# Animesh005/Torus-FHE

Measured on AMD Instinct MI355X. Metric: bootstrapped gates/sec (NAND, N=1024), higher is better.
Workload: dtype f64

## Files before the change

torus-fhe_amd/csrc/thfhe_common.h:

```cpp
#ifndef THFHE_COMMON_H
#define THFHE_COMMON_H

#include <hip/hip_runtime.h>

#include <type_traits>

#include "../../include/thfhe_hip.h"
#include "thfhe_lane.h"

namespace thfhe {

constexpr int kOpIdentity = 100;

int thfhe_fail(int code, const char *msg);
int thfhe_fail_hip(hipError_t e, const char *what);

inline int ilog2(int x) {
    int l = 0;
    while ((1 << l) < x) l++;
    return l;
}

inline int lut_validate(const thfhe_lut_spec *sp, const void *tv, int n_luts, const int32_t *lut_index, const int32_t *in0, const int32_t *in1,
                        const int32_t *in2, const int32_t *out, size_t count, int max_luts = 1024) {
// ... 125 lines not shown
                w[r + 1][d] = __builtin_amdgcn_update_dpp(b, a, 0x128, 0xF, 0x3, false);
                w[r][d] = __builtin_amdgcn_update_dpp(a, b, 0x128, 0xF, 0xC, false);
            }
        }
    }
    if constexpr (KEEP64) {
#pragma unroll
        for (int r = 0; r < 8; r += 2) {
#pragma unroll
            for (int k = 0; k < 2; k++) {
                uint64_t keep = (uint64_t)w[r + 1][2 * k] | (uint64_t)w[r + 1][2 * k + 1] << 32;
                asm("" : "+v"(keep));
#pragma unroll
                for (int h = 0; h < 2; h++) {
                    const int d = 2 * k + h;
                    const uint32_t a = w[r][d], b = w[r + 1][d], kept = (uint32_t)(keep >> (32 * h));
                    w[r + 1][d] = __builtin_amdgcn_update_dpp(b, a, 0x128, 0xF, 0x3, false);
                    w[r][d] = __builtin_amdgcn_update_dpp(a, kept, 0x128, 0xF, 0xC, false);
                }
            }
        }
    }
#pragma unroll
    for (int r = 0; r < 8; r++) __builtin_memcpy(&z[r], w[r], 16);
}
__device__ __forceinline__ void wave_fft_fwd_q(int lane, cplx (&z)[8], cplx *xb, const LaneRoots &r, const W64 &w) {
    fwdq_seg1(z, r);
    wave_transpose_hi3(z);
    wave_sync();
    fwdr_seg2_st(lane, z, xb, w);
    wave_sync();
    fwd_seg3(lane, z, xb);
}
template <bool FLIPPED>
__device__ __forceinline__ void wave_transpose_x3(cplx (&z)[8]) {
    uint32_t w[8][4];
#pragma unroll
    for (int r = 0; r < 8; r++) __builtin_memcpy(w[r], &z[r], 16);
    if constexpr (FLIPPED) {
#pragma unroll
        for (int r = 4; r < 8; r++)
#pragma unroll
            for (int d = 0; d < 4; d++) w[r][d] = __builtin_amdgcn_update_dpp(w[r][d], w[r][d], 0x128, 0xF, 0xF, false);
    } else {
#pragma unroll
        for (int r = 0; r < 4; r++) {
#pragma unroll
            for (int k = 0; k < 2; k++) {
                uint64_t keep = (uint64_t)w[r + 4][2 * k] | (uint64_t)w[r + 4][2 * k + 1] << 32;
                asm("" : "+v"(keep));
#pragma unroll
                for (int h = 0; h < 2; h++) {
                    const int d = 2 * k + h;
                    const uint32_t a = w[r][d], b = w[r + 4][d], kept = (uint32_t)(keep >> (32 * h));
                    w[r + 4][d] = __builtin_amdgcn_update_dpp(b, a, 0x128, 0xF, 0x3, false);
                    w[r][d] = __builtin_amdgcn_update_dpp(a, kept, 0x128, 0xF, 0xC, false);
                }
            }
        }
    }
#pragma unroll
    for (int d = 0; d < 4; d++) {
#pragma unroll
        for (int r = 0; r < 8; r++) {
            if (r & 2) continue;
            auto q = __builtin_amdgcn_permlane32_swap(w[r][d], w[r + 2][d], false, false);
            w[r][d] = q[0];
            w[r + 2][d] = q[1];
        }
#pragma unroll
        for (int r = 0; r < 8; r += 2) {
            auto q = __builtin_amdgcn_permlane16_swap(w[r][d], w[r + 1][d], false, false);
            w[r][d] = q[0];
            w[r + 1][d] = q[1];
        }
    }
#pragma unroll
    for (int r = 0; r < 8; r++) __builtin_memcpy(&z[r], w[r], 16);
}
__device__ __forceinline__ void wave_fft_fwd_x(int lane, cplx (&z)[8], cplx *xb, const LaneRootsF &r) {
    fwdf_seg1(z);
    wave_transpose_x3<false>(z);
    wave_sync();
    fwdx_seg2_st(lane, z, xb, r);
    wave_sync();
    fwdf_seg3(lane, z, xb, r);
}
template <bool LEAN>
__device__ __forceinline__ void wave_fft_inv_x(int lane, cplx (&z)[8], cplx *xb, W64 &w, LaneRoots &r, uint32_t flip, const cplx (&bc)[4]) {
    if (LEAN) opaque_in_place(w.w1), opaque_in_place(r.s);
    wave_sync();
    invf_seg1(lane, z, xb);
    wave_sync();
    inv_seg2_ld(lane, z, xb);
    invf_seg2(z, w);
    wave_transpose_x3<true>(z);
    invx_seg3(z, r, flip, bc);
}
__device__ __forceinline__ void wave_fft_fwd_qs(int lane, cplx (&z)[8], cplx *xb, const LaneRoots &r, const W64 &w) {
    fwdq_seg1(z, r);
    wave_transpose_hi3(z);
    wave_sync();
    fwds_seg2_st(lane, z, xb, w);
    wave_sync();
    fwds_seg3(lane, z, xb);
}
__device__ __forceinline__ void wave_fft_inv_qs(int lane, cplx (&z)[8], cplx *xb, const LaneRoots &r, const W64 &w) {
    wave_sync();
    invs_seg1(lane, z, xb, w);
    wave_sync();
    invs_seg2_ld(lane, z, xb);
    dft8<-1>(z);
    wave_transpose_hi3(z);
    invq_seg3(z, r);
}
template <int T>
__device__ __forceinline__ void wave_fft_fwd_t(int lane, cplx (&z)[8], cplx *xb, const cplx *T1t, const W64 &w) {
    wave_sync();
    fwdt_seg1<T>(lane, z, xb, T1t);
    wave_sync();
    fwds_seg2_ld(lane, z, xb);
    fwds_seg2_st(lane, z, xb, w);
    wave_sync();
    fwds_seg3(lane, z, xb);
}
template <int T>
__device__ __forceinline__ void wave_fft_inv_t(int lane, cplx (&z)[8], cplx *xb, const cplx *T1t, const W64 &w) {
    wave_sync();
    invs_seg1(lane, z, xb, w);
    wave_sync();
// ... 62 lines not shown
```

torus-fhe_amd/csrc/thfhe_lane.h:

```cpp
#ifndef THFHE_LANE_H
#define THFHE_LANE_H

#include <limits.h>
#include <stddef.h>
#include <stdint.h>

#if defined(__HIPCC__)
#define THFHE_FN __host__ __device__ __forceinline__
#else
#define THFHE_FN inline __attribute__((always_inline))
#endif

namespace thfhe {

constexpr int kLanes = 64;
constexpr int kXbufSlots = 8 * 72;

struct alignas(16) cplx {
    double re, im;
};

THFHE_FN cplx cmul(cplx a, cplx b) { return cplx{a.re * b.re - a.im * b.im, a.re * b.im + a.im * b.re}; }
THFHE_FN cplx cmul_conj(cplx a, cplx b) {
    return cplx{a.re * b.re + a.im * b.im, a.im * b.re - a.re * b.im};
// ... 349 lines not shown
}
THFHE_FN W64 lane_w64_x(cplx w64_j0, uint32_t flip) { return W64{cplx{flip_sign(w64_j0.re, flip), flip_sign(w64_j0.im, flip)}}; }
template <typename WPtr>
THFHE_FN LaneRoots lane_roots_x(const WPtr tw, int t1_base, int roots_base, int lane) {
    const int nu = lane_nu(lane);
    return LaneRoots{(lane & 8) ? tw[t1_base + 4 * 64 + nu] : tw[roots_base + 2 * nu], tw[roots_base + 2 * nu + 1]};
}
THFHE_FN void make_untwist_x(cplx b, uint32_t flip, cplx (&bc)[4]) {
    make_untwist_f(b, bc);
    bc[1] = cplx{flip_sign(bc[1].re, flip), flip_sign(bc[1].im, flip)};
    bc[3] = cplx{flip_sign(bc[3].re, flip), flip_sign(bc[3].im, flip)};
}
THFHE_FN constexpr int fwdx_phys(int j1) { return ((j1 & 1) << 2) | ((j1 >> 2) & 1) << 1 | ((j1 >> 1) & 1); }
THFHE_FN void fwdx_seg2_st(int lane, cplx (&z)[8], cplx *xbuf, const LaneRootsF &r) {
    cplx y[8];
#pragma unroll
    for (int j1 = 0; j1 < 8; j1++) y[j1] = z[fwdx_phys(j1)];
    dft8_tw<+1>(y, root_powers<+1>(r.s));
#pragma unroll
    for (int k1 = 0; k1 < 8; k1++) xbuf[xs_c(k1, lane)] = y[k1];
}
THFHE_FN void invx_seg3(cplx (&z)[8], const LaneRoots &r, uint32_t flip, const cplx (&bc)[4]) {
    constexpr double R = 0.70710678118654752440;
    RootPow p = root_powers<-1>(cconj(r.s));
    p.w4.im = flip_sign(p.w4.im, flip);
    dft8_tw<-1>(z, p);
#pragma unroll
    for (int m = 0; m < 4; m++) {
        z[m] = cmul_conj(z[m], bc[m]);
        z[m + 4] = cmul_conj(cplx{R * (z[m + 4].re + z[m + 4].im), R * (z[m + 4].im - z[m + 4].re)}, bc[m]);
    }
}

THFHE_FN uint32_t rot_minus_self32(const int32_t *p, int q, int a2n, int N) {
    int e = (q - a2n) & (2 * N - 1);
    uint32_t r = (uint32_t)p[e & (N - 1)];
    if (e & N) r = 0u - r;
    return r - (uint32_t)p[q];
}
THFHE_FN double digit32(uint32_t v, int shift, uint32_t mask, int32_t half) {
    return (double)((int32_t)((v >> shift) & mask) - half);
}
THFHE_FN uint32_t decomp_offset32(int l, int Bgbit) {
    uint32_t off = 0;
    for (int p = 1; p <= l; p++) off += (1u << (Bgbit - 1)) << (32 - p * Bgbit);
    return off;
}
THFHE_FN uint32_t round_lo32(double x) {
    double y = x + 6755399441055744.0;
    uint64_t b;
    __builtin_memcpy(&b, &y, 8);
    return (uint32_t)b;
}
THFHE_FN void split_limbs32(int32_t v, double &lo, double &hi) {
    int32_t l = (int32_t)(int16_t)(uint16_t)v;
    int32_t h = (int32_t)(((int64_t)v - l) >> 16);
    lo = (double)l;
    hi = (double)h;
}

THFHE_FN int32_t modswitch2n(int32_t x, int log2_2n) {
    int32_t y = (int32_t)((uint32_t)x + (1u << (32 - log2_2n - 1)));
    return y >> (32 - log2_2n);
}


// ... 153 lines not shown
    s.im = __builtin_fma(z.im, b.re, s.im);
}
THFHE_FN void cfma_negkey(cplx &s, cplx z, cplx b) {
    s.re = __builtin_fma(z.re, b.re, s.re);
    s.im = __builtin_fma(z.re, b.im, s.im);
    s.re = __builtin_fma(z.im, -b.im, s.re);
    s.im = __builtin_fma(z.im, b.re, s.im);
}
template <int DEPTH = 8>
THFHE_FN void mac8(int lane, cplx (&S)[8], const cplx (&z)[8], const cplx *B) {
#pragma unroll
    for (int m0 = 0; m0 < 8; m0 += DEPTH) {
        cplx b[DEPTH];
#pragma unroll
        for (int q = 0; q < DEPTH; q++) b[q] = B[(m0 + q) * 64 + lane];
#pragma unroll
        for (int q = 0; q < DEPTH; q++) cfma(S[m0 + q], z[m0 + q], b[q]);
    }
}
THFHE_FN void load8(int lane, cplx (&b)[8], const cplx *B) {
#pragma unroll
    for (int m = 0; m < 8; m++) b[m] = B[m * 64 + lane];
}
THFHE_FN void mac8r(cplx (&S)[8], const cplx (&z)[8], const cplx (&b)[8]) {
#pragma unroll
    for (int m = 0; m < 8; m++) cfma(S[m], z[m], b[m]);
}
THFHE_FN void acc_update16(int lane, int32_t *acc_poly, const cplx (&zlo)[8], const cplx (&zhi)[8]) {
#pragma unroll
    for (int m = 0; m < 8; m++) {
        int q = lane + 64 * m;
        uint32_t vr = round_lo32(zlo[m].re) + (round_lo32(zhi[m].re) << 16);
        uint32_t vi = round_lo32(zlo[m].im) + (round_lo32(zhi[m].im) << 16);
        acc_poly[q] = (int32_t)((uint32_t)acc_poly[q] + vr);
        acc_poly[q + 512] = (int32_t)((uint32_t)acc_poly[q + 512] + vi);
    }
}
THFHE_FN void acc_init16(int lane, int32_t *acc_mask, int32_t *acc_body, int barb, int32_t mu) {
#pragma unroll
    for (int m = 0; m < 16; m++) {
        int q = lane + 64 * m;
        int e = (q + barb) & 2047;
        acc_mask[q] = 0;
        acc_body[q] = (e & 1024) ? (int32_t)(0u - (uint32_t)mu) : mu;
    }
}
THFHE_FN void extract16(int lane, const int32_t *acc_mask, const int32_t *acc_body, int32_t *out) {
#pragma unroll
    for (int m = 0; m < 16; m++) {
        int q = lane + 64 * m;
        out[q] = q == 0 ? acc_mask[0] : (int32_t)(0u - (uint32_t)acc_mask[1024 - q]);
    }
    if (lane == 0) out[1024] = acc_body[0];
}
THFHE_FN void acc_init_tv16(int lane, int32_t *acc_mask, int32_t *acc_body, int barb, const int32_t *tv) {
#pragma unroll
    for (int m = 0; m < 16; m++) {
        int q = lane + 64 * m;
        int e = (q + barb) & 2047;
        const int32_t v = tv[e & 1023];
        acc_mask[q] = 0;
        acc_body[q] = (e & 1024) ? (int32_t)(0u - (uint32_t)v) : v;
    }
}
THFHE_FN void acc_init_tlwe16(int lane, int32_t *acc_mask, int32_t *acc_body, int barb, const int32_t *tv_a, const int32_t *tv_b) {
#pragma unroll
// ... 60 lines not shown
THFHE_FN uint64_t decomp_offset64(int l, int Bgbit) {
    uint64_t off = 0;
    for (int p = 1; p <= l; p++) off += (1ull << (Bgbit - 1)) << (64 - p * Bgbit);
    return off;
}
THFHE_FN void load_rotated16_hi(int lane, const int64_t *acc_poly, int a2n, uint64_t offset, uint32_t (&t)[16]) {
#pragma unroll
    for (int m = 0; m < 16; m++) t[m] = (uint32_t)((rot_minus_self64(acc_poly, lane + 64 * m, a2n) + offset) >> 32);
}
THFHE_FN void split_limbs64(int64_t v, double (&l)[4]) {
#pragma unroll
    for (int q = 0; q < 3; q++) {
        int64_t lo = (int64_t)(int16_t)(uint16_t)v;
        l[q] = (double)lo;
        v = (v - lo) >> 16;
    }
    l[3] = (double)v;
}
template <int TB>
THFHE_FN cplx limb_pair(const void *poly, int q0, int q1, int h) {
    if (TB == 32) {
        const int32_t *p = static_cast<const int32_t *>(poly);
        double l0, h0, l1, h1;
        split_limbs32(p[q0], l0, h0);
        split_limbs32(p[q1], l1, h1);
        return h == 0 ? cplx{l0, l1} : cplx{h0, h1};
    } else {
        const int64_t *p = static_cast<const int64_t *>(poly);
        double a[4], b[4];
        split_limbs64(p[q0], a);
        split_limbs64(p[q1], b);
        return cplx{a[h], b[h]};
    }
}
THFHE_FN void key_limbs64_to_z(int lane, const int64_t *poly, cplx (&z)[4][8]) {
#pragma unroll
    for (int h = 0; h < 4; h++)
#pragma unroll
        for (int m = 0; m < 8; m++) z[h][m] = limb_pair<64>(poly, lane + 64 * m, lane + 64 * m + 512, h);
}
THFHE_FN void key_limbs64_to_z16(int lane, const int64_t *poly, int h, cplx (&z)[16]) {
#pragma unroll
    for (int m = 0; m < 16; m++) z[m] = limb_pair<64>(poly, lane + 64 * m, lane + 64 * m + 1024, h);
}
THFHE_FN int64_t round_i64(double x) {
    double y = x + 6755399441055744.0;
    int64_t b;
    __builtin_memcpy(&b, &y, 8);
    return b - 0x4338000000000000ll;
}
THFHE_FN void acc_update16_64(int lane, int64_t *acc_poly, const cplx (&S)[4][8]) {
#pragma unroll
    for (int m = 0; m < 8; m++) {
        int q = lane + 64 * m;
        uint64_t vr = 0, vi = 0;
#pragma unroll
        for (int h = 0; h < 4; h++) {
            vr += (uint64_t)round_i64(S[h][m].re) << (16 * h);
            vi += (uint64_t)round_i64(S[h][m].im) << (16 * h);
        }
        acc_poly[q] = (int64_t)((uint64_t)acc_poly[q] + vr);
        acc_poly[q + 512] = (int64_t)((uint64_t)acc_poly[q + 512] + vi);
    }
}
THFHE_FN void acc_init16_64(int lane, int64_t *acc_mask, int64_t *acc_body, int barb, int64_t mu) {
#pragma unroll
// ... 319 lines not shown
```

torus-fhe_amd/csrc/thfhe_sk.hip:

```cpp
#include <hip/hip_runtime.h>

#include <algorithm>
#include <memory>
#include <mutex>
#include <new>
#include <string>
#include <vector>

#include "../../include/thfhe_hip.h"
#include "thfhe_cb.h"
#include "thfhe_common.h"
#include "thfhe_dag.h"
#include "thfhe_devctx.h"
#include "thfhe_keyswitch.h"
#include "thfhe_lane.h"
#include "thfhe_launch_plan.h"
#include "thfhe_pack.h"
#include "thfhe_pbs_host.h"
#include "thfhe_ring_schedule.h"

using namespace thfhe;

namespace {

// ... 18 lines not shown
    case THFHE_ORYN: L = Lin{E8, 1, -1, 1}; return true;
    case THFHE_MUX: L = which == 0 ? Lin{-E8, 1, 1, 1} : Lin{-E8, -1, 1, 2}; return true;
    case kOpIdentity: L = Lin{0, 1, 0, 1}; return true;
    default: return false;
    }
}

__global__ __launch_bounds__(256) void sk_prologue_kernel(const int32_t *__restrict__ in0, const int32_t *__restrict__ in1,
                                                           const int32_t *__restrict__ in2, int op, const int32_t *__restrict__ ops,
                                                           int rot_per_gate, int n, int n_pad, int log2_2n, long jobs,
                                                           int32_t *__restrict__ bara, int32_t *__restrict__ barb) {
    const long job = blockIdx.y;
    const int i = blockIdx.x * 256 + threadIdx.x;
    if (job >= jobs || i > n) return;
    const long gate = job / rot_per_gate;
    const int which = (int)(job % rot_per_gate);
    Lin L;
    gate_lin(ops ? ops[gate] : op, which, L);
    const size_t off = (size_t)gate * (n + 1) + i;
    uint32_t v = (uint32_t)L.cx * (uint32_t)in0[off];
    if (L.cy != 0) v += (uint32_t)L.cy * (uint32_t)(L.ysel == 2 ? in2[off] : in1[off]);
    if (i == n) {
        v += (uint32_t)L.cb;
        barb[job] = modswitch2n((int32_t)v, log2_2n);
    } else {
        bara[job * n_pad + i] = modswitch2n((int32_t)v, log2_2n);
    }
}

THFHE_STAMP_STORAGE

struct BRArgs {
    const cplx *bk;
    const cplx *tw;
    const int32_t *bara;
    const int32_t *barb;
    int32_t *out;
    long jobs;
    int n, n_pad, Bgbit;
    int32_t mu;
    const int32_t *tv;
    const int32_t *lut_idx;
    int theta;
    const int32_t *tv_a;
    const int32_t *mv_w;
    int mv_p, mv_box;
};

constexpr int kGate = 0, kLut = 1, kLutEnc = 2, kLutMv = 3;

template <int L, int W = 8, int LUT = kGate>
__global__ __launch_bounds__(64 * W, W == 8 ? 2 : 1) void sk_blind_rotate_ring_kernel(BRArgs a) {
    __shared__ __attribute__((aligned(4096))) int32_t sAcc[W][2048];
    __shared__ cplx sX[W][kXbufSlots];
    __shared__ cplx sRing[3][512];
    constexpr int ROWS = 2 * L;
    constexpr int DPC = 8 / W;
    namespace RS = ring_schedule;
    const int wave = __builtin_amdgcn_readfirstlane(threadIdx.x >> 6);
    const int lane = threadIdx.x & 63;
    const int nu = lane_nu(lane);
    const uint32_t flip = lane_flip_x(lane);
    W64 w64 = lane_w64_x(a.tw[TwRing1k::T2 + 1 * 8 + (lane & 7)], flip);
    LaneRoots roots = lane_roots_x(a.tw, TwRing1k::T1, TwRing1k::ROOTS, lane);
    LaneRootsF rootsf{a.tw[TwRing1k::ROOTSF + 2 * nu], a.tw[TwRing1k::ROOTSF + 2 * nu + 1]};
    const long job = (long)blockIdx.x * W + wave;
    const bool has_job = job < a.jobs;
    int32_t *acc = sAcc[wave];
    cplx *xb = sX[wave];
    const uniform_i32_ptr bara = as_uniform(a.bara + (has_job ? job : 0) * a.n_pad);
    const int Bgbit = a.Bgbit;
    if (has_job) {
        if constexpr (LUT == kLutEnc) {
            const size_t t = a.lut_idx ? (size_t)a.lut_idx[job] * 1024 : 0;
            acc_init_tlwe16(lane, acc, acc + 1024, a.barb[job], a.tv_a + t, a.tv + t);
        } else if constexpr (LUT == kLutMv) acc_init_tv16(lane, acc, acc + 1024, a.barb[job], a.tv);
        else if constexpr (LUT) acc_init_tv16(lane, acc, acc + 1024, a.barb[job], a.tv + (a.lut_idx ? (size_t)a.lut_idx[job] * 1024 : 0));
        else acc_init16(lane, acc, acc + 1024, a.barb[job], a.mu);
    }

    static_assert(DPC == 1 || DPC == 2, "a wave brings one slice of a chunk, or two 1 KiB apart");
    const uint32_t lane_off = (uint32_t)(wave * (64 * DPC) + lane) * (uint32_t)sizeof(cplx);
    uint64_t gbase = (uint64_t)(size_t)a.bk;
    int chunks_ahead = a.n * ROWS * RS::kChunksPerRow - 1;
    asm volatile("" : "+s"(gbase), "+s"(chunks_ahead));
    static_assert(RS::kResidentSlots * RS::kSlotBytes == sizeof(sRing) && RS::kSlotBytes <= sizeof(sX[0]), "ring schedule against the LDS layout");
    const uint32_t ring_base = (uint32_t)(size_t)(__attribute__((address_space(3))) void *)&sRing[0][0] + (uint32_t)wave * (1024u * DPC);
    const uint32_t lent_base = (uint32_t)(size_t)(__attribute__((address_space(3))) void *)&sX[0][0] + (uint32_t)wave * (1024u * DPC);
    auto issue = [&](int slot) {
        const uint32_t dst = slot == RS::kBorrowedSlot ? lent_base : ring_base + (uint32_t)slot * (uint32_t)RS::kSlotBytes;
        ring_dma(gbase, lane_off, dst);
        if constexpr (DPC == 2) ring_dma<1024>(gbase, lane_off, dst);
        gbase += chunks_ahead > 0 ? (uint32_t)RS::kSlotBytes : 0u;
        chunks_ahead = chunks_ahead > 0 ? chunks_ahead - 1 : 0;
    };
    auto slot_ptr = [&](int slot) -> const cplx * { return slot == RS::kBorrowedSlot ? &sX[0][0] : &sRing[slot][0]; };
    __syncthreads();
#pragma unroll
    for (int k = 0; k < RS::kPrologueIssues; k++) issue(RS::kPlan[k].slot);
    STAMP_DECL;

    for (int i = 0; i < a.n; i++) {
        const int ai = bara[i];
        const bool active = has_job && ai != 0;
        const int a2n = ai & 2047;
        cplx S[2][2][8];
#pragma unroll
        for (int c = 0; c < 2; c++)
#pragma unroll
            for (int h = 0; h < 2; h++)
#pragma unroll
                for (int m = 0; m < 8; m++) S[c][h][m] = cplx{0.0, 0.0};
        constexpr int NF = 16;
        uint32_t fld[NF];
#pragma unroll
        for (int r = 0; r < ROWS; r++) {
            cplx z[8];
            if (active) {
                int a2n_r = a2n;
                asm volatile("" : "+s"(a2n_r));
                if (r % L == 0) rotated_fields_keep<NF, W == 4>(lane, acc + (r / L) * 1024, a2n_r, L, Bgbit, fld);
                asm volatile("" : "+s"(a2n_r));
                mixed_digits_z<NF>(lane, acc + (r / L) * 1024, a2n_r, (r % L) + 1, L, Bgbit, fld, z);
                if (W == 8) opaque_in_place(rootsf.s), opaque_in_place(rootsf.w);
                wave_fft_fwd_x(lane, z, xb, rootsf);
            }
            STAMP(0);
            cplx bA[4], bB[4];
            auto consume = [&](int c4) {
                const cplx *B = slot_ptr(RS::kPlan[c4].slot);
                if (active) {
#pragma unroll
                    for (int m = 0; m < 4; m++) bA[m] = B[m * 64 + nu];
                    if (c4 > 0) {
#pragma unroll
                        for (int m = 0; m < 4; m++) cfma_negkey(S[(c4 - 1) >> 1][(c4 - 1) & 1][4 + m], z[4 + m], bB[m]);
                    }
#pragma unroll
                    for (int m = 0; m < 4; m++) bB[m] = B[(4 + m) * 64 + nu];
#pragma unroll
                    for (int m = 0; m < 4; m++) cfma_negkey(S[c4 >> 1][c4 & 1][m], z[m], bA[m]);
                }
            };
            ring_barrier<RS::vmcnt_at(RS::kBarA) * DPC>();
            STAMP(1);
#pragma unroll
            for (int k = 0; k < RS::issues_at(RS::kBarA); k++) issue(RS::issue_slot(RS::kBarA, k));
#pragma unroll
            for (int c4 = RS::first_consumed(RS::kBarA); c4 < RS::first_consumed(RS::kBarX); c4++) consume(c4);
            STAMP(2);
            ring_barrier<RS::vmcnt_at(RS::kBarX) * DPC>();
            STAMP(1);
#pragma unroll
            for (int k = 0; k < RS::issues_at(RS::kBarX); k++) issue(RS::issue_slot(RS::kBarX, k));
#pragma unroll
            for (int c4 = RS::first_consumed(RS::kBarX); c4 < RS::first_consumed(RS::kBarB); c4++) consume(c4);
            STAMP(2);
            ring_barrier<RS::vmcnt_at(RS::kBarB) * DPC>();
            static_assert(RS::issues_at(RS::kBarB) == 0 && RS::first_consumed(RS::kBarB) == RS::kChunksPerRow, "nothing is issued or read after barrier B");
            STAMP(1);
            if (active) {
#pragma unroll
                for (int m = 0; m < 4; m++) cfma_negkey(S[1][1][4 + m], z[4 + m], bB[m]);
            }
            STAMP(2);
        }
        if (active) {
            wave_sync();
            cplx bc[4];
            if (W == 8) opaque_in_place(roots.b);
            make_untwist_x(roots.b, flip, bc);
#pragma unroll
            for (int c = 0; c < 2; c++) {
                wave_fft_inv_x<W == 8>(lane, S[c][0], xb, w64, roots, flip, bc);
                wave_fft_inv_x<W == 8>(lane, S[c][1], xb, w64, roots, flip, bc);
                acc_update16(nu, acc + c * 1024, S[c][0], S[c][1]);
            }
            wave_sync();
        }
        STAMP(3);
    }
    STAMP_FLUSH(blockIdx.x, wave);
    asm volatile("s_waitcnt vmcnt(0)" ::: "memory");
    if (has_job) {
        if constexpr (LUT == kLutMv) {
            const uniform_i32_ptr w = as_uniform(a.mv_w) + (size_t)(a.lut_idx ? as_uniform(a.lut_idx)[job] : 0) * a.theta * a.mv_p;
            for (int j = 0; j < a.theta; j++) extract_mv16(lane, acc, acc + 1024, w + j * a.mv_p, a.mv_p, a.mv_box, a.out + (job * a.theta + j) * 1025);
        } else if constexpr (LUT) {
            for (int j = 0; j < a.theta; j++) extract_at16(lane, acc, acc + 1024, j, a.out + (job * a.theta + j) * 1025);
        } else {
            extract16(lane, acc, acc + 1024, a.out + job * 1025);
        }
    }
}

__device__ __forceinline__ void wg_barrier() { asm volatile("s_waitcnt lgkmcnt(0)\n\ts_barrier" ::: "memory"); }
__device__ __forceinline__ void pin() { asm volatile("" ::: "memory"); }

template <int L, int LUT = kGate>
__global__ __launch_bounds__(512, 2) void sk_blind_rotate_coop_kernel(BRArgs a) {
    constexpr int ROWS = 2 * L;
    __shared__ __attribute__((aligned(4096))) int32_t sAcc[2048];
    __shared__ cplx sSpec[ROWS][512];
    __shared__ cplx sX[8][kXbufSlots];
    const int wave = __builtin_amdgcn_readfirstlane(threadIdx.x >> 6);
    const int lane = threadIdx.x & 63;
    const W64 w64{a.tw[TwRing1k::T2 + 1 * 8 + (lane & 7)]};
    const LaneRoots roots{a.tw[TwRing1k::ROOTS + 2 * lane], a.tw[TwRing1k::ROOTS + 2 * lane + 1]};
    const long job = blockIdx.x;
// ... 103 lines not shown
        STAMP(5);
        i = inext;
    }
    STAMP_FLUSH(blockIdx.x, wave);
    if constexpr (LUT == kLutMv) {
        const uniform_i32_ptr w = as_uniform(a.mv_w) + (size_t)(a.lut_idx ? as_uniform(a.lut_idx)[job] : 0) * a.theta * a.mv_p;
        for (int j = wave; j < a.theta; j += 8)
            extract_mv16(lane, sAcc, sAcc + 1024, w + j * a.mv_p, a.mv_p, a.mv_box, a.out + (job * a.theta + j) * 1025);
    } else if constexpr (LUT) {
        if (wave < a.theta) extract_at16(lane, sAcc, sAcc + 1024, wave, a.out + (job * a.theta + wave) * 1025);
    } else {
        if (wave == 0) extract16(lane, sAcc, sAcc + 1024, a.out + job * 1025);
    }
}

__global__ __launch_bounds__(256) void sk_linear_kernel(const int32_t *__restrict__ in0, int32_t *__restrict__ out, size_t words, int negate) {
    const size_t q = (size_t)blockIdx.x * 256 + threadIdx.x;
    if (q < words) out[q] = negate ? (int32_t)(0u - (uint32_t)in0[q]) : in0[q];
}

}

struct THFHE_INTERNAL thfhe_tgsw_set {
    thfhe_ctx *ctx = nullptr;
    DevBuf spec;
    size_t count = 0;
    int d = 0;
};

struct THFHE_INTERNAL thfhe_ctx : DevCtx {
    thfhe_params p;
    int rec_words() const { return p.n + 1; }
    DevBuf d_bk;
    KsKey ksk;
    int coop_max_jobs = 768;
    int ring4_max_jobs = 1024;
    int n_pad = 0;
    DevBuf d_bara, d_barb, d_u;
    DevBuf d_tv, d_lut_idx;
    DevBuf d_tva;
    DevBuf d_mv_w;
    DevBuf d_tree_tab, d_tree_lwe, d_tree_a, d_tree_b;
    DevBuf d_dag_enc_a, d_dag_enc_b, d_dag_tv1;
    DevBuf d_dag_mv_tv0, d_dag_mv_w;
    DevBuf d_dag_lhe_tab_a, d_dag_lhe_tab_b, d_dag_lhe_fin_a, d_dag_lhe_fin_b, d_dag_lhe_words;
    DevBuf d_lhe_a, d_lhe_b, d_lhe_in[4];
    DevBuf d_wfa_tab;
    DevBuf d_sc_tab, d_sc_idx;
    CbKey cb;
    std::vector<std::unique_ptr<thfhe_tgsw_set>> cb_sets;
    std::vector<const thfhe_tgsw_set *> dag_sets;
    DevBuf d_cb_lwe, d_cb_bara, d_cb_barb, d_cb_acc, d_cb_x, d_cb_lwe2, d_cb_rows, d_cb_tv;
    int cus = 0;
    int wfa_chunk = 0;
    size_t tree_slice = 65536;
    Stage stage;
    LinBufs lin;
    DagBuffers dag;
    size_t dag_slice = 28672;
    hipEvent_t grp_ev[2] = {nullptr, nullptr};
    bool grp_valid = false;
    ~thfhe_ctx() {
        for (hipEvent_t e : grp_ev)
            if (e) (void)hipEventDestroy(e);
    }
};
// ... 25 lines not shown
    auto piece = [&](long first, long count) {
        BRArgs b = a;
        b.bara += first * a.n_pad, b.barb += first, b.jobs = count;
        b.out += first * (LUT ? a.theta : 1) * 1025;
        if (LUT && b.lut_idx) b.lut_idx += first;
        return b;
    };
    launch_plan::SkPiece pc[launch_plan::kMaxPieces];
    const int n = launch_plan::sk_rotation_plan(a.jobs, coop_max, ring4_max, pc);
    for (int i = 0; i < n; i++) {
        const BRArgs b = piece(pc[i].first, pc[i].count);
        if (pc[i].shape == launch_plan::kRing8) launch_ring8<L, LUT>(b, s);
        else if (pc[i].shape == launch_plan::kCoop) launch_coop<L, LUT>(b, s);
        else launch_ring4<L, LUT>(b, s);
    }
}

template <int LUT>
int launch_rotations(thfhe_ctx *c, const BRArgs &a) {
    return with_static_int<4>(c->p.l, kBadL, [&](auto l) { launch_br<decltype(l)::value, LUT>(a, c->stream, c->coop_max_jobs, c->ring4_max_jobs); });
}

int enqueue_rotations(thfhe_ctx *c, int op, const int32_t *d0, const int32_t *d1, const int32_t *d2, size_t gates,
                      int rot_per_gate, int32_t mu, const int32_t *d_ops = nullptr) {
    const size_t jobs = gates * rot_per_gate;
    int rc = ensure_workspace(c, jobs);
    if (rc) return rc;
    const int n = c->p.n;
    if (c->profiling) THFHE_HIP(hipEventRecord(c->ev[0], c->stream));
    dim3 pg((unsigned)((n + 1 + 255) / 256), (unsigned)jobs);
    hipLaunchKernelGGL(sk_prologue_kernel, pg, dim3(256), 0, c->stream, d0, d1, d2, op, d_ops, rot_per_gate, n, c->n_pad,
                       ilog2(2 * c->p.N), (long)jobs, c->d_bara.as<int32_t>(), c->d_barb.as<int32_t>());
    if (c->profiling) THFHE_HIP(hipEventRecord(c->ev[1], c->stream));
    BRArgs a{c->d_bk.as<cplx>(), c->d_tw.as<cplx>(), c->d_bara.as<int32_t>(), c->d_barb.as<int32_t>(), c->d_u.as<int32_t>(), (long)jobs, n, c->n_pad, c->p.Bgbit, mu};
    rc = launch_rotations<kGate>(c, a);
    if (rc) return rc;
    if (c->profiling) THFHE_HIP(hipEventRecord(c->ev[2], c->stream));
    THFHE_HIP(hipGetLastError());
    return THFHE_OK;
}

int enqueue_keyswitch(thfhe_ctx *c, const int32_t *d_u, int32_t *d_out, size_t gates, int rot_per_gate, bool timed) {
    KsArgs k = c->ksk.args(d_u, d_out, (long)gates);
    k.rot_per_gate = rot_per_gate;
    const int nsplit = gates <= 32 ? 16 : (gates <= 128 ? 8 : (gates <= 512 ? 2 : 1));
    THFHE_TRY(ks_enqueue(c->ksk, k, nsplit, c->stream));
    if (timed && c->profiling) {
        THFHE_HIP(hipEventRecord(c->ev[3], c->stream));
        c->ev_valid = true;
    }
    return THFHE_OK;
}

struct MvArgs {
    const int32_t *w;
    int p;
};

template <typename Src>
int enqueue_pbs(thfhe_ctx *c, const Src &src, size_t jobs, const int32_t *tv, const int32_t *tv_a, int theta, const int32_t *d_idx, int32_t *ks_dst,
                bool timed = false, const MvArgs *mv = nullptr) {
    const int n = c->p.n;
    const bool ev = timed && c->profiling;
    int32_t *const idx = c->d_lut_idx.as<int32_t>();
    if (ev) THFHE_HIP(hipEventRecord(c->ev[0], c->stream));
    lut_prologue_launch(src, jobs, n, c->n_pad, ilog2(2 * c->p.N), c->d_bara.as<int32_t>(), c->d_barb.as<int32_t>(), idx, c->stream);
    if (ev) THFHE_HIP(hipEventRecord(c->ev[1], c->stream));
    BRArgs a{c->d_bk.as<cplx>(), c->d_tw.as<cplx>(), c->d_bara.as<int32_t>(), c->d_barb.as<int32_t>(), c->d_u.as<int32_t>(), (long)jobs, n, c->n_pad, c->p.Bgbit,
             0, tv, Src::kIdx == LutIdx::none ? d_idx : idx, theta, tv_a};
    if (mv) {
        a.mv_w = mv->w, a.mv_p = mv->p, a.mv_box = c->p.N / mv->p;
        THFHE_TRY(launch_rotations<kLutMv>(c, a));
    } else THFHE_TRY(tv_a ? launch_rotations<kLutEnc>(c, a) : launch_rotations<kLut>(c, a));
    if (ev) THFHE_HIP(hipEventRecord(c->ev[2], c->stream));
    THFHE_HIP(hipGetLastError());
    return ks_dst ? enqueue_keyswitch(c, c->d_u.as<int32_t>(), ks_dst, jobs * theta, 1, timed) : THFHE_OK;
}

int gates_dev_locked(thfhe_ctx *c, int op, const int32_t *d0, const int32_t *d1, const int32_t *d2, int32_t *dout, size_t count) {
    if (count == 0) return THFHE_OK;
    if (count > (size_t)INT32_MAX / 4) return thfhe_fail(THFHE_E_INVALID, "count too large");
    THFHE_HIP(hipSetDevice(c->device));
    if (op == THFHE_NOT || op == THFHE_COPY) {
        const size_t words = count * c->rec_words();
        hipLaunchKernelGGL(sk_linear_kernel, dim3((unsigned)((words + 255) / 256)), dim3(256), 0, c->stream, d0, dout, words,
                           op == THFHE_NOT ? 1 : 0);
        THFHE_HIP(hipGetLastError());
        return THFHE_OK;
    }
    Lin L;
    if (!gate_lin(op, 0, L) || op == kOpIdentity) return thfhe_fail(THFHE_E_INVALID, "unknown gate opcode");
    if (!d0 || !d1 || (op == THFHE_MUX && !d2)) return thfhe_fail(THFHE_E_INVALID, "null operand");
    const int rot = op == THFHE_MUX ? 2 : 1;
    int rc = enqueue_rotations(c, op, d0, d1, d2, count, rot, 1 << 29);
    if (rc) return rc;
    return enqueue_keyswitch(c, c->d_u.as<int32_t>(), dout, count, rot, true);
}

int dag_gate_class(thfhe_ctx *c, int cls, const int32_t *d_ops, size_t n) {
    const bool is_mux = cls == kDagMux;
    int r = enqueue_rotations(c, is_mux ? THFHE_MUX : THFHE_NAND, c->stage.in_ptr(0), c->stage.in_ptr(1), is_mux ? c->stage.in_ptr(2) : nullptr, n, is_mux ? 2 : 1, 1 << 29,
// ... 253 lines not shown
int thfhe_device_count(void) {
    int n = 0;
    if (hipGetDeviceCount(&n) != hipSuccess) return 0;
    return n;
}

int thfhe_device_pci_bus_id(int device, char *buf, int len) {
    if (!buf || len < 16) return thfhe_fail(THFHE_E_INVALID, "buffer of at least 16 bytes expected");
    THFHE_HIP(hipDeviceGetPCIBusId(buf, len, device));
    return THFHE_OK;
}

int thfhe_ctx_create(const thfhe_params *p, const int32_t *bk_coeff, const int32_t *ksk, int device, thfhe_ctx **out) {
    if (!p || !bk_coeff || !ksk || !out) return thfhe_fail(THFHE_E_INVALID, "null argument");
    *out = nullptr;
    if (p->torus_bits != 32 || p->parties != 1) return thfhe_fail(THFHE_E_UNSUPPORTED, "thfhe_ctx_create is the single-key Torus32 path; use thfhe_mk_ctx_create");
    if (p->N != 1024 || p->k != 1) return thfhe_fail(THFHE_E_UNSUPPORTED, "only N = 1024, k = 1 is implemented");
    if (p->l < 1 || p->l > 4 || p->Bgbit < 1 || p->Bgbit > 10 || p->l * p->Bgbit > 32)
        return thfhe_fail(THFHE_E_UNSUPPORTED, "need 1 <= l <= 4, Bgbit <= 10 (FP64 exactness bound), l*Bgbit <= 32");
    if (p->n < 1 || p->n > 1407) return thfhe_fail(THFHE_E_UNSUPPORTED, "need 1 <= n <= 1407");
    if (p->ks_t < 1 || p->ks_basebit < 1 || p->ks_t * p->ks_basebit > 31) return thfhe_fail(THFHE_E_INVALID, "bad key-switch parameters");
    std::unique_ptr<thfhe_ctx> c(new (std::nothrow) thfhe_ctx);
    if (!c) return thfhe_fail(THFHE_E_NOMEM, "out of host memory");
    THFHE_TRY(c->open(device, true));
    c->p = *p;
    c->n_pad = (p->n + 3) & ~3;
    THFHE_TRY(c->upload_twiddles(1024));
    DevBuf coeff;
    const long npolys = (long)p->n * 2 * p->l * 2;
    THFHE_TRY(coeff.grow((size_t)npolys * 1024 * sizeof(int32_t)));
    THFHE_HIP(hipMemcpyAsync(coeff.as<int32_t>(), bk_coeff, (size_t)npolys * 1024 * sizeof(int32_t), hipMemcpyHostToDevice, c->stream));
    THFHE_TRY(c->d_bk.grow((size_t)npolys * 1024 * sizeof(cplx)));
    THFHE_TRY((launch_torus_transform<1024, 32>(c->stream, coeff.as<int32_t>(), npolys, c->d_tw.as<cplx>(), c->d_bk.as<cplx>())));
    THFHE_TRY(c->ksk.upload(ksk, 1, p->N, p->n, p->ks_t, p->ks_basebit, true, c->stream));
    *out = c.release();
    return THFHE_OK;
}

void thfhe_ctx_destroy(thfhe_ctx *c) { ctx_destroy(c); }

int thfhe_ctx_params(const thfhe_ctx *c, thfhe_params *out) {
    if (!c || !out) return thfhe_fail(THFHE_E_INVALID, "null argument");
    *out = c->p;
    return THFHE_OK;
}

void *thfhe_dev_alloc(thfhe_ctx *c, size_t bytes) { return ctx_dev_alloc(c, bytes); }
void thfhe_dev_free(thfhe_ctx *c, void *p) { ctx_dev_free(c, p); }
int thfhe_copy_h2d(thfhe_ctx *c, void *dst, const void *src, size_t bytes) { return ctx_copy(c, dst, src, bytes, hipMemcpyHostToDevice); }
int thfhe_copy_d2h(thfhe_ctx *c, void *dst, const void *src, size_t bytes) { return ctx_copy(c, dst, src, bytes, hipMemcpyDeviceToHost); }
int thfhe_reserve(thfhe_ctx *c, size_t max_count) {
    if (!c) return thfhe_fail(THFHE_E_INVALID, "null ctx");
    DevLock lk(*c);
    if (lk.rc) return lk.rc;
    return ensure_workspace(c, max_count * 2);
}
int thfhe_sync(thfhe_ctx *c) { return ctx_sync(c); }
#ifdef THFHE_STAMPS
int thfhe_debug_read_stamps(unsigned long long *dst, size_t count) {
    return hipMemcpyFromSymbol(dst, HIP_SYMBOL(g_stamps), count * sizeof(unsigned long long)) == hipSuccess ? 0 : -1;
}
#endif
int thfhe_set_coop_threshold(thfhe_ctx *c, int max_jobs) {
    if (!c || max_jobs < 0) return thfhe_fail(THFHE_E_INVALID, "bad argument");
    std::lock_guard<std::mutex> g(c->mu);
    c->coop_max_jobs = max_jobs;
// ... 347 lines not shown
```

torus-fhe_amd/csrc/thfhe_transform.h:

```cpp
#ifndef THFHE_TRANSFORM_H
#define THFHE_TRANSFORM_H

struct MapIdentity {
    __device__ long src(long p) const { return p; }
    __device__ size_t dst(long p, int h, int limbs) const { return (size_t)p * limbs + h; }
};

template <int NN, int TB, class Map>
__global__ __launch_bounds__(256) void torus_transform_kernel(const void *__restrict__ torus, long npolys, const cplx *__restrict__ tw,
                                                              cplx *__restrict__ spec, Map map) {
    constexpr int LIMBS = TB / 16;
    __shared__ cplx sT1[NN == 2048 ? 2 : 1][512];
    __shared__ cplx sX[4][512];
    if constexpr (NN == 1024) {
        for (int t = threadIdx.x; t < 512; t += 256) sT1[0][t] = tw[TwRing1k::T1 + t];
        __syncthreads();
    } else if constexpr (NN == 2048) {
        for (int t = threadIdx.x; t < 512; t += 256) {
            sT1[0][t] = tw[TwRing2k::T1_TWIST1 + t];
            sT1[1][t] = tw[TwRing2k::T1_TWIST5 + t];
        }
        __syncthreads();
    }
    const int wave = threadIdx.x >> 6, lane = threadIdx.x & 63;
    const W64 w64{tw[tw_t2<NN>() + 1 * 8 + (lane & 7)]};
    const long item = (long)blockIdx.x * 4 + wave;
    if (item >= npolys * LIMBS) return;
    const long p = item / LIMBS;
    const int h = (int)(item % LIMBS);
    const char *poly = static_cast<const char *>(torus) + (size_t)map.src(p) * NN * (TB / 8);
    cplx *dst = spec + map.dst(p, h, LIMBS) * (NN / 2);
    if constexpr (NN == 1024) {
        cplx z[8];
#pragma unroll
        for (int m = 0; m < 8; m++) z[m] = limb_pair<TB>(poly, lane + 64 * m, lane + 64 * m + 512, h);
        wave_fft_fwd_s(lane, z, sX[wave], sT1[0], w64);
#pragma unroll
        for (int m = 0; m < 8; m++) dst[m * 64 + lane] = cplx{z[m].re * (1.0 / 512), z[m].im * (1.0 / 512)};
    } else if constexpr (NN == 2048) {
        cplx z[16], y0[8], y1[8];
#pragma unroll
        for (int m = 0; m < 16; m++) z[m] = limb_pair<TB>(poly, lane + 64 * m, lane + 64 * m + 1024, h);
        split2048(z, y0, y1);
        wave_fft_fwd_t<1>(lane, y0, sX[wave], sT1[0], w64);
        wave_fft_fwd_t<5>(lane, y1, sX[wave], sT1[1], w64);
#pragma unroll
        for (int m = 0; m < 8; m++) {
            dst[m * 64 + lane] = cplx{y0[m].re * (1.0 / 1024), y0[m].im * (1.0 / 1024)};
            dst[512 + m * 64 + lane] = cplx{y1[m].re * (1.0 / 1024), y1[m].im * (1.0 / 1024)};
        }
    } else {
        static_assert(NN == 4096, "ring degrees 1024, 2048 and 4096");
        const cplx ratio = tw[TwRing2k::RATIO + lane];
#pragma unroll
        for (int qt = 0; qt < 4; qt++) {
            cplx y[8];
#pragma unroll
            for (int m = 0; m < 8; m++) {
                cplx u[4];
#pragma unroll
                for (int s = 0; s < 4; s++) u[s] = limb_pair<TB>(poly, lane + 64 * m + 512 * s, lane + 64 * m + 512 * s + 2048, h);
                pre4096(u);
                y[m] = qt == 0 ? comb4096<0>(u) : qt == 1 ? comb4096<1>(u) : qt == 2 ? comb4096<2>(u) : comb4096<3>(u);
            }
            const LaneRoots roots{tw[TwRing2k::ROOTS4K + qt * 64 + lane], ratio};
            if (qt == 0) wave_fft_fwd_tq<1, 64>(lane, y, sX[wave], roots, w64);
            if (qt == 1) wave_fft_fwd_tq<5, 64>(lane, y, sX[wave], roots, w64);
            if (qt == 2) wave_fft_fwd_tq<9, 64>(lane, y, sX[wave], roots, w64);
            if (qt == 3) wave_fft_fwd_tq<13, 64>(lane, y, sX[wave], roots, w64);
// ... 41 lines not shown
```

Baseline: 146,800.

## Use phased bootstrapping-key copy to simplify ring FFT transposes and scaling

```diff
diff --git a/torus-fhe_amd/csrc/thfhe_common.h b/torus-fhe_amd/csrc/thfhe_common.h
--- a/torus-fhe_amd/csrc/thfhe_common.h
+++ b/torus-fhe_amd/csrc/thfhe_common.h
@@ -181,33 +181,14 @@
     wave_sync();
     fwd_seg3(lane, z, xb);
 }
-template <bool FLIPPED>
 __device__ __forceinline__ void wave_transpose_x3(cplx (&z)[8]) {
     uint32_t w[8][4];
 #pragma unroll
     for (int r = 0; r < 8; r++) __builtin_memcpy(w[r], &z[r], 16);
-    if constexpr (FLIPPED) {
-#pragma unroll
-        for (int r = 4; r < 8; r++)
-#pragma unroll
-            for (int d = 0; d < 4; d++) w[r][d] = __builtin_amdgcn_update_dpp(w[r][d], w[r][d], 0x128, 0xF, 0xF, false);
-    } else {
-#pragma unroll
-        for (int r = 0; r < 4; r++) {
-#pragma unroll
-            for (int k = 0; k < 2; k++) {
-                uint64_t keep = (uint64_t)w[r + 4][2 * k] | (uint64_t)w[r + 4][2 * k + 1] << 32;
-                asm("" : "+v"(keep));
-#pragma unroll
-                for (int h = 0; h < 2; h++) {
-                    const int d = 2 * k + h;
-                    const uint32_t a = w[r][d], b = w[r + 4][d], kept = (uint32_t)(keep >> (32 * h));
-                    w[r + 4][d] = __builtin_amdgcn_update_dpp(b, a, 0x128, 0xF, 0x3, false);
-                    w[r][d] = __builtin_amdgcn_update_dpp(a, kept, 0x128, 0xF, 0xC, false);
-                }
-            }
-        }
-    }
+#pragma unroll
+    for (int r = 4; r < 8; r++)
+#pragma unroll
+        for (int d = 0; d < 4; d++) w[r][d] = __builtin_amdgcn_update_dpp(w[r][d], w[r][d], 0x128, 0xF, 0xF, false);
 #pragma unroll
     for (int d = 0; d < 4; d++) {
 #pragma unroll
@@ -227,11 +208,11 @@
 #pragma unroll
     for (int r = 0; r < 8; r++) __builtin_memcpy(&z[r], w[r], 16);
 }
-__device__ __forceinline__ void wave_fft_fwd_x(int lane, cplx (&z)[8], cplx *xb, const LaneRootsF &r) {
-    fwdf_seg1(z);
-    wave_transpose_x3<false>(z);
-    wave_sync();
-    fwdx_seg2_st(lane, z, xb, r);
+__device__ __forceinline__ void wave_fft_fwd_x(int lane, cplx (&z)[8], cplx *xb, const LaneRootsF &r, uint32_t flip) {
+    fwdp_seg1(z, flip);
+    wave_transpose_x3(z);
+    wave_sync();
+    fwdp_seg2_st(lane, z, xb, r, flip);
     wave_sync();
     fwdf_seg3(lane, z, xb, r);
 }
@@ -243,8 +224,8 @@
     wave_sync();
     inv_seg2_ld(lane, z, xb);
     invf_seg2(z, w);
-    wave_transpose_x3<true>(z);
-    invx_seg3(z, r, flip, bc);
+    wave_transpose_x3(z);
+    invx_seg3_ring(z, r, flip, bc);
 }
 __device__ __forceinline__ void wave_fft_fwd_qs(int lane, cplx (&z)[8], cplx *xb, const LaneRoots &r, const W64 &w) {
     fwdq_seg1(z, r);
diff --git a/torus-fhe_amd/csrc/thfhe_lane.h b/torus-fhe_amd/csrc/thfhe_lane.h
--- a/torus-fhe_amd/csrc/thfhe_lane.h
+++ b/torus-fhe_amd/csrc/thfhe_lane.h
@@ -405,6 +405,35 @@
     }
 }
 
+THFHE_FN void invx_seg3_ring(cplx (&z)[8], const LaneRoots &r, uint32_t flip, const cplx (&bc)[4]) {
+    RootPow p = root_powers<-1>(cconj(r.s));
+    p.w4.im = flip_sign(p.w4.im, flip);
+    dft8_tw<-1>(z, p);
+#pragma unroll
+    for (int m = 0; m < 4; m++) {
+        z[m] = cmul_conj(z[m], bc[m]);
+        z[m + 4] = cmul_conj(cplx{z[m + 4].re + z[m + 4].im, z[m + 4].im - z[m + 4].re}, bc[m]);
+    }
+}
+
+THFHE_FN cplx flip_sign(cplx v, uint32_t flip) { return cplx{flip_sign(v.re, flip), flip_sign(v.im, flip)}; }
+THFHE_FN void fwdp_seg1(cplx (&z)[8], uint32_t flip) {
+#pragma unroll
+    for (int m = 0; m < 4; m++) bfly_c4(z[m], z[m + 4]);
+    z[5] = flip_sign(z[5], flip);
+    z[7] = flip_sign(z[7], flip);
+    dft8_tw_tail<+1>(z, flip_sign(cplx{THFHE_C_RE(1), THFHE_C_IM(1)}, flip), cplx{THFHE_C_RE(2), THFHE_C_IM(2)}, cplx{THFHE_C_RE(5), THFHE_C_IM(5)});
+}
+THFHE_FN void fwdp_seg2_st(int lane, cplx (&z)[8], cplx *xbuf, const LaneRootsF &r, uint32_t flip) {
+    RootPow p = root_powers<+1>(r.s);
+    p.w4.im = flip_sign(p.w4.im, flip);
+    dft8_tw<+1>(z, p);
+#pragma unroll
+    for (int k1 = 0; k1 < 8; k1++) xbuf[xs_c(k1, lane)] = z[k1];
+}
+constexpr int kKeyPhase = 32;
+THFHE_FN bool key_point_phased(int nu) { return (nu & 32) != 0; }
+
 THFHE_FN uint32_t rot_minus_self32(const int32_t *p, int q, int a2n, int N) {
     int e = (q - a2n) & (2 * N - 1);
     uint32_t r = (uint32_t)p[e & (N - 1)];
@@ -624,6 +653,22 @@
         int q = lane + 64 * m;
         uint32_t vr = round_lo32(zlo[m].re) + (round_lo32(zhi[m].re) << 16);
         uint32_t vi = round_lo32(zlo[m].im) + (round_lo32(zhi[m].im) << 16);
+        acc_poly[q] = (int32_t)((uint32_t)acc_poly[q] + vr);
+        acc_poly[q + 512] = (int32_t)((uint32_t)acc_poly[q + 512] + vi);
+    }
+}
+THFHE_FN uint32_t round_scaled_lo32(double x) {
+    double y = __builtin_fma(0.70710678118654752440, x, 6755399441055744.0);
+    uint64_t b;
+    __builtin_memcpy(&b, &y, 8);
+    return (uint32_t)b;
+}
+THFHE_FN void acc_update16_ring(int lane, int32_t *acc_poly, const cplx (&zlo)[8], const cplx (&zhi)[8]) {
+#pragma unroll
+    for (int m = 0; m < 8; m++) {
+        const int q = lane + 64 * m;
+        const uint32_t vr = m < 4 ? round_lo32(zlo[m].re) + (round_lo32(zhi[m].re) << 16) : round_scaled_lo32(zlo[m].re) + (round_scaled_lo32(zhi[m].re) << 16);
+        const uint32_t vi = m < 4 ? round_lo32(zlo[m].im) + (round_lo32(zhi[m].im) << 16) : round_scaled_lo32(zlo[m].im) + (round_scaled_lo32(zhi[m].im) << 16);
         acc_poly[q] = (int32_t)((uint32_t)acc_poly[q] + vr);
         acc_poly[q + 512] = (int32_t)((uint32_t)acc_poly[q + 512] + vi);
     }
@@ -750,6 +795,14 @@
         split_limbs64(p[q1], b);
         return cplx{a[h], b[h]};
     }
+}
+THFHE_FN cplx limb_pair_rot32(const int32_t *p, int q0, int q1, int h, int rot) {
+    const int e0 = (q0 - rot) & 2047, e1 = (q1 - rot) & 2047;
+    double l0, h0, l1, h1;
+    split_limbs32(p[e0 & 1023], l0, h0);
+    split_limbs32(p[e1 & 1023], l1, h1);
+    const double a = h == 0 ? l0 : h0, b = h == 0 ? l1 : h1;
+    return cplx{(e0 & 1024) ? -a : a, (e1 & 1024) ? -b : b};
 }
 THFHE_FN void key_limbs64_to_z(int lane, const int64_t *poly, cplx (&z)[4][8]) {
 #pragma unroll
diff --git a/torus-fhe_amd/csrc/thfhe_sk.hip b/torus-fhe_amd/csrc/thfhe_sk.hip
--- a/torus-fhe_amd/csrc/thfhe_sk.hip
+++ b/torus-fhe_amd/csrc/thfhe_sk.hip
@@ -74,6 +74,7 @@
 
 struct BRArgs {
     const cplx *bk;
+    const cplx *bk_ring;
     const cplx *tw;
     const int32_t *bara;
     const int32_t *barb;
@@ -123,7 +124,7 @@
 
     static_assert(DPC == 1 || DPC == 2, "a wave brings one slice of a chunk, or two 1 KiB apart");
     const uint32_t lane_off = (uint32_t)(wave * (64 * DPC) + lane) * (uint32_t)sizeof(cplx);
-    uint64_t gbase = (uint64_t)(size_t)a.bk;
+    uint64_t gbase = (uint64_t)(size_t)a.bk_ring;
     int chunks_ahead = a.n * ROWS * RS::kChunksPerRow - 1;
     asm volatile("" : "+s"(gbase), "+s"(chunks_ahead));
     static_assert(RS::kResidentSlots * RS::kSlotBytes == sizeof(sRing) && RS::kSlotBytes <= sizeof(sX[0]), "ring schedule against the LDS layout");
@@ -161,11 +162,11 @@
             if (active) {
                 int a2n_r = a2n;
                 asm volatile("" : "+s"(a2n_r));
-                if (r % L == 0) rotated_fields_keep<NF, W == 4>(lane, acc + (r / L) * 1024, a2n_r, L, Bgbit, fld);
+                if (r % L == 0) rotated_fields_keep<NF, W == 4>(nu, acc + (r / L) * 1024, a2n_r, L, Bgbit, fld);
                 asm volatile("" : "+s"(a2n_r));
-                mixed_digits_z<NF>(lane, acc + (r / L) * 1024, a2n_r, (r % L) + 1, L, Bgbit, fld, z);
+                mixed_digits_z<NF>(nu, acc + (r / L) * 1024, a2n_r, (r % L) + 1, L, Bgbit, fld, z);
                 if (W == 8) opaque_in_place(rootsf.s), opaque_in_place(rootsf.w);
-                wave_fft_fwd_x(lane, z, xb, rootsf);
+                wave_fft_fwd_x(lane, z, xb, rootsf, flip);
             }
             STAMP(0);
             cplx bA[4], bB[4];
@@ -216,7 +217,7 @@
             for (int c = 0; c < 2; c++) {
                 wave_fft_inv_x<W == 8>(lane, S[c][0], xb, w64, roots, flip, bc);
                 wave_fft_inv_x<W == 8>(lane, S[c][1], xb, w64, roots, flip, bc);
-                acc_update16(nu, acc + c * 1024, S[c][0], S[c][1]);
+                acc_update16_ring(nu, acc + c * 1024, S[c][0], S[c][1]);
             }
             wave_sync();
         }
@@ -386,6 +387,7 @@
     thfhe_params p;
     int rec_words() const { return p.n + 1; }
     DevBuf d_bk;
+    DevBuf d_bk_ring;
     KsKey ksk;
     int coop_max_jobs = 768;
     int ring4_max_jobs = 1024;
@@ -477,7 +479,7 @@
     hipLaunchKernelGGL(sk_prologue_kernel, pg, dim3(256), 0, c->stream, d0, d1, d2, op, d_ops, rot_per_gate, n, c->n_pad,
                        ilog2(2 * c->p.N), (long)jobs, c->d_bara.as<int32_t>(), c->d_barb.as<int32_t>());
     if (c->profiling) THFHE_HIP(hipEventRecord(c->ev[1], c->stream));
-    BRArgs a{c->d_bk.as<cplx>(), c->d_tw.as<cplx>(), c->d_bara.as<int32_t>(), c->d_barb.as<int32_t>(), c->d_u.as<int32_t>(), (long)jobs, n, c->n_pad, c->p.Bgbit, mu};
+    BRArgs a{c->d_bk.as<cplx>(), c->d_bk_ring.as<cplx>(), c->d_tw.as<cplx>(), c->d_bara.as<int32_t>(), c->d_barb.as<int32_t>(), c->d_u.as<int32_t>(), (long)jobs, n, c->n_pad, c->p.Bgbit, mu};
     rc = launch_rotations<kGate>(c, a);
     if (rc) return rc;
     if (c->profiling) THFHE_HIP(hipEventRecord(c->ev[2], c->stream));
@@ -511,7 +513,7 @@
     if (ev) THFHE_HIP(hipEventRecord(c->ev[0], c->stream));
     lut_prologue_launch(src, jobs, n, c->n_pad, ilog2(2 * c->p.N), c->d_bara.as<int32_t>(), c->d_barb.as<int32_t>(), idx, c->stream);
     if (ev) THFHE_HIP(hipEventRecord(c->ev[1], c->stream));
-    BRArgs a{c->d_bk.as<cplx>(), c->d_tw.as<cplx>(), c->d_bara.as<int32_t>(), c->d_barb.as<int32_t>(), c->d_u.as<int32_t>(), (long)jobs, n, c->n_pad, c->p.Bgbit,
+    BRArgs a{c->d_bk.as<cplx>(), c->d_bk_ring.as<cplx>(), c->d_tw.as<cplx>(), c->d_bara.as<int32_t>(), c->d_barb.as<int32_t>(), c->d_u.as<int32_t>(), (long)jobs, n, c->n_pad, c->p.Bgbit,
              0, tv, Src::kIdx == LutIdx::none ? d_idx : idx, theta, tv_a};
     if (mv) {
         a.mv_w = mv->w, a.mv_p = mv->p, a.mv_box = c->p.N / mv->p;
@@ -831,6 +833,8 @@
     THFHE_HIP(hipMemcpyAsync(coeff.as<int32_t>(), bk_coeff, (size_t)npolys * 1024 * sizeof(int32_t), hipMemcpyHostToDevice, c->stream));
     THFHE_TRY(c->d_bk.grow((size_t)npolys * 1024 * sizeof(cplx)));
     THFHE_TRY((launch_torus_transform<1024, 32>(c->stream, coeff.as<int32_t>(), npolys, c->d_tw.as<cplx>(), c->d_bk.as<cplx>())));
+    THFHE_TRY(c->d_bk_ring.grow((size_t)npolys * 1024 * sizeof(cplx)));
+    THFHE_TRY((launch_torus_transform<1024, 32, MapPhased>(c->stream, coeff.as<int32_t>(), npolys, c->d_tw.as<cplx>(), c->d_bk_ring.as<cplx>())));
     THFHE_TRY(c->ksk.upload(ksk, 1, p->N, p->n, p->ks_t, p->ks_basebit, true, c->stream));
     *out = c.release();
     return THFHE_OK;
diff --git a/torus-fhe_amd/csrc/thfhe_transform.h b/torus-fhe_amd/csrc/thfhe_transform.h
--- a/torus-fhe_amd/csrc/thfhe_transform.h
+++ b/torus-fhe_amd/csrc/thfhe_transform.h
@@ -5,6 +5,14 @@
     __device__ long src(long p) const { return p; }
     __device__ size_t dst(long p, int h, int limbs) const { return (size_t)p * limbs + h; }
 };
+
+struct MapPhased : MapIdentity {
+    static constexpr bool kPhased = true;
+};
+template <class Map, class = void>
+struct map_is_phased : std::false_type {};
+template <class Map>
+struct map_is_phased<Map, std::void_t<decltype(Map::kPhased)>> : std::true_type {};
 
 template <int NN, int TB, class Map>
 __global__ __launch_bounds__(256) void torus_transform_kernel(const void *__restrict__ torus, long npolys, const cplx *__restrict__ tw,
@@ -35,6 +43,17 @@
 #pragma unroll
         for (int m = 0; m < 8; m++) z[m] = limb_pair<TB>(poly, lane + 64 * m, lane + 64 * m + 512, h);
         wave_fft_fwd_s(lane, z, sX[wave], sT1[0], w64);
+        if constexpr (map_is_phased<Map>::value) {
+            static_assert(TB == 32, "the phased copy is the single-key ring kernels'");
+            cplx y[8];
+#pragma unroll
+            for (int m = 0; m < 8; m++) y[m] = limb_pair_rot32(reinterpret_cast<const int32_t *>(poly), lane + 64 * m, lane + 64 * m + 512, h, kKeyPhase);
+            wave_fft_fwd_s(lane, y, sX[wave], sT1[0], w64);
+            if (key_point_phased(lane)) {
+#pragma unroll
+                for (int m = 0; m < 8; m++) z[m] = y[m];
+            }
+        }
 #pragma unroll
         for (int m = 0; m < 8; m++) dst[m * 64 + lane] = cplx{z[m].re * (1.0 / 512), z[m].im * (1.0 / 512)};
     } else if constexpr (NN == 2048) {
```

Result: faster. 148,500, median of 6 (+1.1%).
